# vlaxose/jstsp19

Hardware: AMD Instinct MI355X
Metric: channel-estimates/sec (batched MC) at Nt=Nr=64,K=64; NMSE vs ref (higher is better)
Workload: dtype c32 (storage and results fp32 complex; big contractions as split-f16 MFMA with fp32 accumulation, fp32-equivalent); 1 GPU; proposed_algorithm approximate Imax=100, Nt=Nr=64 Nrf=8 K=64 L=8 (N=64 M=4096 Gr=64 G2=512); Imax=100, outputs=S,Y,convergence_error, pilots=per-trial (B per trial), parallelism=trials sharded, dp1

## Files before the change

### jstsp19_amd/csrc/common.h

```cpp
#pragma once
#include <hip/hip_runtime.h>
#include <cstdint>
#include <cstdio>
#include <cstdarg>
#include <string>
#include <vector>
#include <map>
#include "../../include/jstsp.h"

namespace jstsp {

void set_error(const char *fmt, ...);

#define JSTSP_HIP(call)                                                                  \
    do {                                                                                 \
        hipError_t e_ = (call);                                                          \
        if (e_ != hipSuccess) {                                                          \
            jstsp::set_error("%s failed: %s (%s:%d)", #call, hipGetErrorString(e_),      \
                             __FILE__, __LINE__);                                        \
            return (int)e_;                                                              \
        }                                                                                \
    } while (0)

#define JSTSP_TRY(expr)                                                                  \
    do {                                                                                 \
        int rc_ = (expr);                                                                \
        if (rc_ != 0) return rc_;                                                        \
    } while (0)

#define JSTSP_REQUIRE(cond, code, ...)                                                   \
    do {                                                                                 \
        if (!(cond)) {                                                                   \
            jstsp::set_error(__VA_ARGS__);                                               \
            return (code);                                                               \
        }                                                                                \
    } while (0)

struct DeviceScope {
    int prev = -1;
    bool switched = false;
    hipError_t err = hipSuccess;
    explicit DeviceScope(int dev)
    {
        err = hipGetDevice(&prev);
        if (err == hipSuccess && prev != dev) {
            err = hipSetDevice(dev);
            switched = (err == hipSuccess);
        }
    }
    ~DeviceScope() { if (switched) (void)hipSetDevice(prev); }
    DeviceScope(const DeviceScope &) = delete;
    DeviceScope &operator=(const DeviceScope &) = delete;
};
struct Tuning {
    int h2 = 1;
    int fused = 1;
    int fused_parts = 0;
    int fused_kback = 4;
    int toeplitz = 2;
    int overlap = -1;
    int lanczos = 1;
    int lanczos_warm = 1;
    int lanczos_verify = 32;
    int eig128 = 1;
    int host_compact = 1;
    int host_pipeline = 1;
    int bj_mask = 1;
};
const Tuning &tune();
void load_tuning();

#define JSTSP_ENTER(ctx)                                                                 \
    jstsp::DeviceScope dev_scope_((ctx)->device);                                        \
    JSTSP_HIP(dev_scope_.err);                                                           \
    jstsp::load_tuning()

struct TrialParams {
    float rho, irho;
    float tauY_rho;
    float tauS_rho;
    float c_coef;
    float rho_lo, irho_lo, c_lo;
    float omc, omc_lo;
    float omr, omr_lo;
    float omir, omir_lo;
    float pad[2];
};
#if defined(__cplusplus)
inline TrialParams make_trial_params(double rho, double tau_Y, double tau_S)
{
    TrialParams p;
    auto split = [](double v, float &h, float &l) { h = (float)v; l = (float)(v - (double)h); };
    split(rho, p.rho, p.rho_lo);
    split(1.0 / rho, p.irho, p.irho_lo);
    split(rho / (rho + 1.0), p.c_coef, p.c_lo);
    split(1.0 / (rho + 1.0), p.omc, p.omc_lo);
    split(1.0 - rho, p.omr, p.omr_lo);
    split(1.0 - 1.0 / rho, p.omir, p.omir_lo);
    p.tauY_rho = (float)(tau_Y / rho);
    p.tauS_rho = (float)(tau_S / rho);
    p.pad[0] = p.pad[1] = 0.f;
    return p;
}
#if defined(__HIPCC__)
__device__ __forceinline__ float mul2(float ch, float cl, float x) { return fmaf(ch, x, cl * x); }
__device__ __forceinline__ float admm_v2(const TrialParams &p, float v2, float x, float xs)
{
    const float dx = x - xs;
    const float t = fmaf(-p.rho, dx, v2) - p.rho_lo * dx;
    return mul2(p.omc, p.omc_lo, t);
}
__device__ __forceinline__ float admm_x(const TrialParams &p, float v1, float y, float sy, float v2, float xs, float invd)
{
    const float ys = y + xs;
    return ((v1 + sy) + mul2(p.rho, p.rho_lo, ys) + mul2(p.omr, p.omr_lo, v2)) * invd;
}
__device__ __forceinline__ float admm_x2(const TrialParams &p, float v1, float y, float sy, float v2, float xs, float rh, float rl)
{
    const float ys = y + xs;
    const float s = (v1 + sy) + mul2(p.rho, p.rho_lo, ys) + mul2(p.omr, p.omr_lo, v2);
    return fmaf(s, rh, s * rl);
}
__device__ __forceinline__ void admm_invd(const TrialParams &p, float om, float &rh, float &rl)
{
    const float a = 2.f * p.rho, al = 2.f * p.rho_lo;
    const float dh = om + a;
    const float bb = dh - om;
    const float dl = ((om - (dh - bb)) + (a - bb)) + al;
    rh = __builtin_amdgcn_rcpf(dh);
    rl = rh * (fmaf(-dh, rh, 1.f) - dl * rh);
}
__device__ __forceinline__ float admm_k(const TrialParams &p, float x, float v2) { return fmaf(p.omir, v2, x) + p.omir_lo * v2; }
__device__ __forceinline__ float admm_v1(const TrialParams &p, float v1, float y, float x)
{
    const float d = y - x;
    return fmaf(p.rho, d, v1) + p.rho_lo * d;
}
__device__ __forceinline__ float admm_z(const TrialParams &p, float x, float v1) { return fmaf(-p.irho, v1, x) - p.irho_lo * v1; }
#endif
#endif

struct Arena {
    char *base = nullptr;
    size_t cap = 0, off = 0;
    int reserve(size_t bytes);
    void reset() { off = 0; }
    template <class T> T *get(size_t n) {
        size_t bytes = (n * sizeof(T) + 255) & ~size_t(255);
        if (off + bytes > cap) return nullptr;
        T *p = reinterpret_cast<T *>(base + off);
        off += bytes;
        return p;
    }
    void release();
};

struct ProfileSlot {
    int launches = 0;
    std::vector<std::pair<hipEvent_t, hipEvent_t>> pending;
    double total_ms = 0;
};

}

struct jstsp_ctx {
    int device = 0;
    hipStream_t stream = nullptr;
    bool own_stream = false;
    jstsp::Arena arena;
    bool profiling = false;
    std::map<std::string, jstsp::ProfileSlot> prof;
    std::vector<hipEvent_t> event_pool;
    int num_cus = 256;
    void *pinned = nullptr;
    size_t pinned_cap = 0, pinned_off = 0;
    hipEvent_t pinned_done = nullptr;
    bool pinned_pending = false;
    uint32_t *diag = nullptr;
    unsigned *lz_mismatch = nullptr;
    void *hpin = nullptr;
    size_t hpin_cap = 0;
    hipEvent_t hpin_done = nullptr;
    bool hpin_pending = false;
    int dict_block_hint = 0;
    int last_dict_block = 0;
    int fused_fallbacks = 0;
    float2 *unit = nullptr;
    double2 *unit64 = nullptr;
    jstsp_ctx *helper = nullptr;
    hipStream_t side[2] = {nullptr, nullptr};
    hipStream_t cu_stream[4] = {nullptr, nullptr, nullptr, nullptr};
    int cu_state = 0;
    hipStream_t bj_stream[3] = {nullptr, nullptr, nullptr};
    hipEvent_t bj_ev[6] = {nullptr, nullptr, nullptr, nullptr, nullptr, nullptr};
    hipEvent_t ev[10] = {nullptr, nullptr, nullptr, nullptr, nullptr, nullptr, nullptr, nullptr, nullptr, nullptr};
};

namespace jstsp {

struct GemmDesc {
    const float2 *A; long long sAt, sAi, sAk; int conjA;
    const float2 *B; long long sBt, sBk, sBj; int conjB;
    const float2 *B2;
    float2 *C; long long sCt; int ldc;
    const float2 *D; long long sDt; int ldd;
    float alpha, beta;
    int m, n, k, batch;
    int splitk; long long sCsplit;
    int epi;
    const TrialParams *prm;
    float2 *e_rw0, *e_w1, *e_w2, *e_w3;
// ... 115 lines not shown
```

### jstsp19_amd/csrc/proposed.hip

```cpp
#include "solver_common.h"
#include <cstdio>
#include <cmath>
#include <cstdlib>
#include <algorithm>

namespace jstsp {

struct ProposedWS {
    float2 *X, *V1, *V2, *C, *Xs, *Y, *ZK, *Zb, *Zb2;
    float *invD;
    float2 *V, *RV, *Res, *RRes, *S, *P1;
    float2 *Tc, *W;
    float2 *GA, *GB;
    TrialParams *prm;
    int32_t *rank;
    double *ce;
    float *lam;
    GramWS gz, gn;
    bool h2 = false;
    HPack Bc, Bs;
    uint32_t *kmax = nullptr, *wmax = nullptr;
    uint32_t *nmax = nullptr, *zmax = nullptr;
    bool h2g = false;
    HPack GBp;
// ... 274 lines not shown
        JSTSP_REQUIRE((PA || GAi) && (PB || GBi), JSTSP_E_NOMEM, "proposed_algorithm 'std': workspace exhausted");
        const size_t mark = ctx->arena.off;
        if (!PA) {
            JSTSP_TRY(hermitian_inverse(ctx, Gr, nA, w.GA, GAi));
            ctx->arena.off = mark;
            JSTSP_HIP(hipMemcpyAsync(w.GA, GAi, (size_t)nA * Gr * Gr * sizeof(float2), hipMemcpyDeviceToDevice, st));
        }
        if (!PB) {
            JSTSP_TRY(hermitian_inverse(ctx, G2, nB, w.GB, GBi));
            ctx->arena.off = mark;
            JSTSP_HIP(hipMemcpyAsync(w.GB, GBi, (size_t)nB * G2 * G2 * sizeof(float2), hipMemcpyDeviceToDevice, st));
        }
    }
    const long long snm = (long long)nm, sg = (long long)g, sng = (long long)ng;
    constexpr int rv_refresh = 4;
    auto refresh_at = [](int it) -> bool { return it % rv_refresh == 0; };
    const bool overlap = tn.overlap >= 0 ? tn.overlap != 0 : want_fused;
    uint32_t *const kmax0 = w.kmax;
    JSTSP_TRY(ensure_side_streams(ctx));
    hipStream_t sm = ctx->stream, s1 = overlap ? ctx->side[0] : sm, s2 = overlap ? ctx->side[1] : sm;
    hipEvent_t ev_x = ctx->ev[0], ev_svt = ctx->ev[1], ev_gxv = ctx->ev[2], ev_c = ctx->ev[3], ev_gv2 = ctx->ev[4],
               ev_ce = ctx->ev[5], ev_lxv = ctx->ev[6];
    if (Imax > 0) {
        JSTSP_TRY(launch_form_z(ctx, snm, batch, w.X, w.V1, w.prm, w.Zb));
        JSTSP_TRY(svt_prepare(ctx, w.gz, w.Zb, w.prm, nullptr, true));
    }
    const bool fz = w.gz.left;
    const bool hmax = w.h2 && fz && N <= 64;
    const bool zfly = hmax && want_ce && gram3_nsplit(N, M, G2, want_ce) > 0 && w.gz.nsplit == w.gn.nsplit;
    float2 *Zbuf[2] = {w.Zb, w.Zb2};
    const bool fusedp = want_fused && hmax && (want_ce ? zfly : true);
    const bool fusedy = fusedp;
    FusedWS fw;
    if (fusedp) {
        if (toep_env != 0 && !toep_probed) JSTSP_TRY(fused_probe_toeplitz(ctx, ctx->arena, B, strideB, G2, M, nB, &toep_gt));
        ctx->last_dict_block = toep_gt;
        JSTSP_TRY(fused_alloc(ctx->arena, fw, M, G2, nB, batch, fparts, toep_gt, toep_env >= 2 && fusedy));
        JSTSP_TRY(fused_pack_b(ctx, fw, B, strideB, G2, M, nB, w.Bc.bmax));
        JSTSP_HIP(hipMemsetAsync(fw.ovf, 0, (size_t)batch * sizeof(uint32_t), sm));
    }
    const int fused_kback = tn.fused_kback;
    bool passed = false;
    hipEvent_t ev_q1 = ctx->ev[7];
    if (want_ce) JSTSP_TRY(lanczos_warm_reset(ctx, w.gn));
    for (int it = 0; it < Imax; ++it) {
        if (want_ce) w.gn.lz.call = it;
        float2 *Zc = fz ? Zbuf[it & 1] : w.Zb, *Zn = fz ? Zbuf[(it + 1) & 1] : w.Zb;
        if (w.h2) {
            const size_t boff = (size_t)(it & 1) * 8 * (size_t)batch;
            w.kmax = kmax0 + boff; w.nmax = w.kmax + batch; w.zmax = w.kmax + 4 * (size_t)batch;
            w.wmax = w.kmax + 5 * (size_t)batch; w.pmax = w.kmax + 6 * (size_t)batch;
            if (!passed) JSTSP_HIP(hipMemsetAsync(w.kmax, 0, 8 * (size_t)batch * sizeof(uint32_t), sm));
        } else if (w.h2g) JSTSP_HIP(hipMemsetAsync(w.pmax, 0, 2 * (size_t)batch * sizeof(uint32_t), sm));
        int apply_no = 0;
        if (it > 0) JSTSP_HIP(hipStreamWaitEvent(sm, ev_svt, 0));
        if (it > 0 && want_ce) JSTSP_HIP(hipStreamWaitEvent(sm, ev_gxv, 0));
        if (passed) {
        } else if (fz) {
            JSTSP_TRY(launch_eye_minus(ctx, N, batch, w.gz.Q, w.gz.Q));
            GemmDesc dq = make_gemm('N', 'N', N, M, N, batch, Mat{w.gz.Q, (long long)N * N, N}, Mat{Zc, snm, N}, w.Y, snm, N);
            dq.epi = EPI_UPDATE_X; dq.prm = w.prm;
            dq.e_rw0 = w.V1; dq.e_w1 = w.X; dq.e_w2 = w.ZK;
            dq.e_r0 = w.V2; dq.e_r2 = w.Xs; dq.e_r3 = subY; dq.e_f0 = w.invD;
            dq.e_w3 = (it + 1 < Imax && (!zfly || fusedy)) ? Zn : nullptr;
            if (zfly && it > 0) { dq.B = w.X; dq.B2 = w.V1; }
            dq.epi_store_c = (it + 1 == Imax);
            if (w.h2) {
                dq.amax_out = w.kmax;
                if (N <= 64) { dq.amax_x = w.nmax; dq.amax_v1 = w.nmax + batch; dq.amax_z = w.zmax; }
            }
            JSTSP_TRY(launch_cgemm(ctx, dq, GEMM_MISC));
        } else {
            JSTSP_TRY(svt_apply(ctx, w.gz, Zc, w.Y));
            JSTSP_TRY(launch_update_x(ctx, snm, batch, w.X, w.V1, w.V2, w.C, w.Xs, w.Y, subY, w.invD, w.prm, w.ZK));
        }
        JSTSP_HIP(hipEventRecord(ev_x, sm));
        auto issue_s1 = [&](int stage) -> int {
            if (stage != 2) JSTSP_HIP(hipStreamWaitEvent(s1, ev_x, 0));
            StreamScope sc(ctx, s1);
            if (stage != 2 && !fz) JSTSP_TRY(launch_form_z(ctx, snm, batch, w.X, w.V1, w.prm, Zn));
            if (zfly) {
              if (stage != 2) {
                if (fusedp && it > 0) JSTSP_HIP(hipStreamWaitEvent(s1, ev_lxv, 0));
                JSTSP_TRY(launch_hgram3(ctx, w.X, w.V1, snm, N, M, batch, w.gz.nsplit, w.nmax, w.nmax + batch, w.zmax,
                                        w.prm, w.gz.Gpart, w.gn.Gpart, w.gn.Gpart + (size_t)batch * N * N * w.gn.nsplit));
                JSTSP_HIP(hipEventRecord(ev_gxv, s1));
                if (fusedp) {
                    JSTSP_HIP(hipStreamWaitEvent(s2, ev_gxv, 0));
                    StreamScope sc2(ctx, s2);
                    JSTSP_TRY(lmax_from_partials_range(ctx, w.gn, 0, 2 * batch, w.lam, true));
                    JSTSP_HIP(hipEventRecord(ev_lxv, s2));
                }
              }
              if (stage == 1) return 0;
                JSTSP_TRY(svt_prepare(ctx, w.gz, w.X, w.prm, nullptr, true, w.zmax, nullptr, true));
                if (fusedy) JSTSP_TRY(fused_pack_wq(ctx, fw, w.gz.Q, batch));
            } else {
                JSTSP_TRY(svt_prepare(ctx, w.gz, Zn, w.prm, nullptr, true, hmax ? w.zmax : nullptr));
                if (fusedy) JSTSP_TRY(fused_pack_wq(ctx, fw, w.gz.Q, batch));
            }
            JSTSP_HIP(hipEventRecord(ev_svt, s1));
            return 0;
        };
        const bool svt_split = passed && fusedp && zfly && it + 1 < Imax;
        if (it + 1 < Imax) JSTSP_TRY(issue_s1(svt_split ? 1 : 0));
        if (want_ce && !(zfly && it + 1 < Imax)) {
            JSTSP_HIP(hipStreamWaitEvent(s2, ev_x, 0));
            StreamScope sc(ctx, s2);
            JSTSP_TRY(gram_partials_range(ctx, w.gn, w.X, snm, 0, 2 * batch, hmax ? w.nmax : nullptr, nullptr, nullptr, true));
            JSTSP_HIP(hipEventRecord(ev_gxv, s2));
        }
        if (passed) {
            JSTSP_TRY(fused_reduce(ctx, fw, G2, M, batch, w.Tc));
        } else if (PB) {
            JSTSP_TRY(gemm(ctx, 'N', 'N', N, G2, M, batch, Mat{w.ZK, snm, N}, Mat{PB, strideB ? (long long)M * G2 : 0, M},
                           w.Tc, sng, N, 1.f, nullptr, 0, 0, 0.f, GEMM_CORRELATE));
        } else if (w.h2) {
            if (!fz) JSTSP_TRY(hgemm_absmax(ctx, w.ZK, snm, snm, batch, w.kmax));
            HGemmDesc hc{w.ZK, snm, N, w.kmax, w.Bc.data, strideB ? w.Bc.st : 0, w.Bc.bmax, strideB ? 1 : 0, w.Bc.KS,
                         w.Bc.JT, w.Tc, sng, N, N, G2, M, batch, EPI_NONE, nullptr, nullptr, nullptr};
            if (w.Kp.data && !strideB && w.Kp.KS == w.Bc.KS) {
                w.Kp.bmax = w.kmax;
                JSTSP_TRY(hgemm_repack(ctx, w.Kp, w.ZK, snm, N, 1, 0, M, N, w.kmax));
                hc.Ap = w.Kp.data; hc.sApt = w.Kp.st; hc.aKS = w.Kp.KS;
            }
            JSTSP_TRY(launch_hgemm(ctx, hc, "correlate"));
        } else
        JSTSP_TRY(gemm(ctx, 'N', 'C', N, G2, M, batch, Mat{w.ZK, snm, N}, Bm, w.Tc, sng, N, 1.f, nullptr, 0, 0,
                       0.f, GEMM_CORRELATE));
        const long long cnt_ll = std::min<long long>(10 + 5ll * (it + 1), (long long)g);
        const Mat GAl{GAlo, strideA ? (long long)Gr * Gr : 0, Gr};
        auto second_factor = [&](float2 *out, uint32_t *pm, bool exact) -> int {
            if (exact || !w.h2g) {
                GemmDesc dr = make_gemm('N', 'N', Gr, G2, G2, batch, Mat{w.P1, sg, Gr}, GBm, out, sg, Gr);
                dr.force_m64 = exact ? 1 : 0;
                return launch_cgemm(ctx, dr, GEMM_MISC);
            }
            HGemmDesc hg{w.P1, sg, Gr, pm, w.GBp.data, strideB ? w.GBp.st : 0, w.GBp.bmax, strideB ? 1 : 0,
                         w.GBp.KS, w.GBp.JT, out, sg, Gr, Gr, G2, G2, batch, EPI_NONE, nullptr, nullptr, nullptr};
            return launch_hgemm(ctx, hg, nullptr);
        };
        auto apply_R = [&](const float2 *Xin, float2 *out, bool exact) -> int {
            uint32_t *pm = w.pmax ? w.pmax + (size_t)(apply_no++ & 1) * batch : nullptr;
            if (exact) JSTSP_TRY(gemm(ctx, 'N', 'N', Gr, G2, Gr, batch, GAl, Mat{Xin, sg, Gr}, w.P1, sg, Gr));
            GemmDesc dp = make_gemm('N', 'N', Gr, G2, Gr, batch, GAm, Mat{Xin, sg, Gr}, w.P1, sg, Gr, 1.f, exact ? w.P1 : nullptr, sg,
                                    Gr, exact ? 1.f : 0.f);
            dp.amax_out = w.h2g ? pm : nullptr;
            JSTSP_TRY(launch_cgemm(ctx, dp, GEMM_MISC));
            return second_factor(out, pm, exact);
        };
        if (approx) {
            const bool refreshed = refresh_at(it);
            if (refreshed) JSTSP_TRY(apply_R(w.V, w.RV, true));
            GemmDesc dres = make_gemm('C', 'N', Gr, G2, N, batch, Am, Mat{w.Tc, sng, N}, w.Res, sg, Gr, 1.f, w.RV, sg, Gr, -1.f);
            JSTSP_TRY(launch_cgemm(ctx, dres, GEMM_MISC));
            JSTSP_TRY(apply_R(w.Res, w.RRes, false));
            if (svt_split) {
                JSTSP_HIP(hipEventRecord(ev_q1, sm));
                JSTSP_HIP(hipStreamWaitEvent(s1, ev_q1, 0));
                JSTSP_TRY(issue_s1(2));
            }
            JSTSP_TRY(launch_step_v(ctx, (int)g, batch, w.Res, w.RRes, w.V, w.S, w.rank, (int)cnt_ll, w.prm, w.ce,
                                    Imax, it, w.RV, svt_split));
        } else {
            float2 *left = PB ? w.V : w.P1;
            if (PA)
                JSTSP_TRY(gemm(ctx, 'N', 'N', Gr, G2, N, batch, Mat{PA, strideA ? (long long)Gr * N : 0, Gr},
                               Mat{w.Tc, sng, N}, left, sg, Gr));
            else {
                JSTSP_TRY(gemm(ctx, 'C', 'N', Gr, G2, N, batch, Am, Mat{w.Tc, sng, N}, w.Res, sg, Gr));
                JSTSP_TRY(gemm(ctx, 'N', 'N', Gr, G2, Gr, batch, GAm, Mat{w.Res, sg, Gr}, left, sg, Gr));
            }
            if (!PB) JSTSP_TRY(gemm(ctx, 'N', 'N', Gr, G2, G2, batch, Mat{w.P1, sg, Gr}, GBm, w.V, sg, Gr));
            JSTSP_TRY(launch_soft(ctx, (int)g, batch, w.V, w.S, w.rank, (int)cnt_ll, w.prm));
        }
        if (fusedp && !want_ce && it + 1 == Imax) break;
        if (w.h2) {
            GemmDesc dw = make_gemm('N', 'N', N, G2, Gr, batch, Am, Mat{w.S, sg, Gr}, w.W, sng, N);
            dw.amax_out = w.wmax;
            JSTSP_TRY(launch_cgemm(ctx, dw, GEMM_MISC));
        } else
        JSTSP_TRY(gemm(ctx, 'N', 'N', N, G2, Gr, batch, Am, Mat{w.S, sg, Gr}, w.W, sng, N));
        if (it > 0 && want_ce) JSTSP_HIP(hipStreamWaitEvent(sm, ev_gv2, 0));
        passed = false;
        if (fusedp && it + 1 < Imax) {
            uint32_t *nx = kmax0 + (size_t)((it + 1) & 1) * 8 * (size_t)batch;
            JSTSP_HIP(hipMemsetAsync(nx, 0, 8 * (size_t)batch * sizeof(uint32_t), sm));
            JSTSP_TRY(fused_pack_as(ctx, fw, w.W, sng, G2, M, batch, w.wmax));
            JSTSP_HIP(hipStreamWaitEvent(sm, ev_svt, 0));
            FusedDesc fd{fw.Bf, strideB ? fw.sBf : 0, w.Bc.bmax, strideB ? 1 : 0, fw.ASp, fw.sAS, w.wmax, w.kmax,
                         w.X, w.V1, w.V2, subY, w.Y, omega_direct ? Omega : w.invD, snm, w.prm, fw.Ppart,
                         nx, nx + batch, nx + 2 * (size_t)batch, nx + 4 * (size_t)batch, w.nmax + 2 * (size_t)batch, fw.ovf,
                         M, G2, batch, fparts,
                         fusedy ? fw.Wqp : nullptr, Zbuf[(it + 1) & 1], w.zmax,
                         (fw.v2 && zfly) ? nullptr : Zbuf[it & 1],
                         (fusedy && it + 2 == Imax) ? w.Y : nullptr, fused_kback,
                         fw.Ec, strideB ? fw.sEc : 0, fw.gt ? 31 - __builtin_clz((unsigned)fw.gt) : 0, fw.ecols, fw.ehalo,
                         fw.v2, fw.XsD, fw.Kf, omega_direct ? 1 : 0};
            JSTSP_TRY(launch_fused_pass(ctx, fd));
            passed = true;
        } else
        if (w.h2) {
            JSTSP_TRY(hgemm_repack(ctx, w.Wp, w.W, sng, N, 1, 0, G2, N, w.wmax));
            if (!w.Bs.data)
                JSTSP_TRY(hgemm_pack(ctx, w.Bs, ctx->arena, B, strideB, 1, G2, 0, G2, M, nB, (long long)G2 * M, w.Bc.bmax));
            HGemmDesc hs{w.W, sng, N, w.wmax, w.Bs.data, strideB ? w.Bs.st : 0, w.Bs.bmax, strideB ? 1 : 0, w.Bs.KS,
                         w.Bs.JT, w.Xs, snm, N, N, M, G2, batch, fz ? EPI_UPDATE_C : EPI_NONE, w.prm, w.X, w.V2,
                         hmax ? w.nmax + 2 * (size_t)batch : nullptr, w.Wp.data, w.Wp.st, w.Wp.KS};
            JSTSP_TRY(launch_hgemm(ctx, hs, "synthesize"));
            if (!fz) JSTSP_TRY(launch_update_c(ctx, snm, batch, w.X, w.Xs, w.V2, w.C, w.prm));
        } else if (fz) {
            GemmDesc ds = make_gemm('N', 'N', N, M, G2, batch, Mat{w.W, sng, N}, Bm, w.Xs, snm, N);
            ds.epi = EPI_UPDATE_C; ds.prm = w.prm;
            ds.e_r0 = w.X; ds.e_rw0 = w.V2;
            JSTSP_TRY(launch_cgemm(ctx, ds, GEMM_SYNTH));
        } else {
            JSTSP_TRY(gemm(ctx, 'N', 'N', N, M, G2, batch, Mat{w.W, sng, N}, Bm, w.Xs, snm, N, 1.f, nullptr, 0, 0,
                           0.f, GEMM_SYNTH));
            JSTSP_TRY(launch_update_c(ctx, snm, batch, w.X, w.Xs, w.V2, w.C, w.prm));
        }
        if (want_ce) {
            JSTSP_HIP(hipEventRecord(ev_c, sm));
            JSTSP_HIP(hipStreamWaitEvent(s2, ev_c, 0));
            if (zfly) JSTSP_HIP(hipStreamWaitEvent(s2, ev_gxv, 0));
            StreamScope sc(ctx, s2);
            JSTSP_TRY(gram_partials_range(ctx, w.gn, w.X, snm, 2 * batch, batch, hmax ? w.nmax : nullptr, nullptr, nullptr, true));
            JSTSP_HIP(hipEventRecord(ev_gv2, s2));
            if (fusedp && zfly && it + 1 < Imax) JSTSP_TRY(lmax_from_partials_range(ctx, w.gn, 2 * batch, batch, w.lam, true));
            else JSTSP_TRY(lmax_from_partials(ctx, w.gn, w.lam, true));
            JSTSP_TRY(launch_ce_ratio(ctx, batch, w.lam + batch, w.lam + 2 * batch, w.lam, w.ce, Imax, it));
            JSTSP_HIP(hipEventRecord(ev_ce, s2));
        }
    }
    if (want_ce && Imax > 0) JSTSP_HIP(hipStreamWaitEvent(sm, ev_ce, 0));
    if (defer) {
        defer->active = true; defer->fused = fusedp; defer->want_ce = want_ce && Imax > 0; defer->batch = batch; defer->g = g; defer->nm = nm;
        defer->Imax = Imax; defer->dS = w.S; defer->dY = w.Y; defer->dce = w.ce; defer->ovf = fusedp ? fw.ovf : nullptr;
        return 0;
    }

    JSTSP_TRY(stage_out(ctx, reinterpret_cast<float2 *>(S_out), w.S, batch * g, memspace));
    JSTSP_TRY(stage_out(ctx, reinterpret_cast<float2 *>(Y_out), w.Y, batch * nm, memspace));
    if (want_ce && Imax > 0) JSTSP_TRY(stage_out(ctx, ce_out, w.ce, (size_t)batch * 3 * Imax, memspace));
    if (fusedp && overflowed) {
        std::vector<uint32_t> flags(batch);
        JSTSP_HIP(hipMemcpyAsync(flags.data(), fw.ovf, (size_t)batch * sizeof(uint32_t), hipMemcpyDeviceToHost, st));
        JSTSP_HIP(hipStreamSynchronize(st));
        for (int t = 0; t < batch; ++t)
            if (flags[t]) overflowed->push_back(t);
    }
    if (memspace == JSTSP_HOST) {
        JSTSP_HIP(hipStreamSynchronize(st));
        if (!approx) JSTSP_TRY(diag_check_host(ctx, "proposed_algorithm 'std'"));
    }
    return 0;
}

static int resolve_overflowed(jstsp_ctx *ctx, const std::vector<int> &ovf, int N, int M, int Gr, int G2, const jstsp_c32 *subY,
                              const float *Omega, const jstsp_c32 *A, long long strideA, const jstsp_c32 *B, long long strideB,
                              int Imax, const double *tau_Y, const double *tau_S, const double *rho, int type,
                              const int32_t *indx_S, jstsp_c32 *S_out, jstsp_c32 *Y_out, double *ce_out, int memspace, int *count)
{
    const size_t nm = (size_t)N * M, g = (size_t)Gr * G2;
    for (size_t i = 0; i < ovf.size();) {
        size_t j = i + 1;
        while (j < ovf.size() && ovf[j] == ovf[j - 1] + 1) ++j;
        const int t0 = ovf[i], cnt = (int)(j - i);
        JSTSP_TRY(proposed_impl(ctx, N, M, Gr, G2, cnt, subY + t0 * nm, Omega + t0 * nm, A + (size_t)t0 * strideA, strideA,
                                B + (size_t)t0 * strideB, strideB, Imax, tau_Y + t0, tau_S + t0, rho + t0, type,
                                indx_S ? indx_S + t0 * g : nullptr, S_out + t0 * g, Y_out ? Y_out + t0 * nm : nullptr,
                                ce_out ? ce_out + (size_t)t0 * 3 * Imax : nullptr, memspace, false, nullptr));
        *count += cnt;
        i = j;
    }
    return 0;
}

static int proposed_finish(jstsp_ctx *ctx, const PendingSolve &p, jstsp_c32 *S_out, jstsp_c32 *Y_out, double *ce_out, std::vector<int> *ovf)
{
    JSTSP_ENTER(ctx);
    JSTSP_TRY(stage_out(ctx, reinterpret_cast<float2 *>(S_out), p.dS, p.batch * p.g, JSTSP_HOST));
    JSTSP_TRY(stage_out(ctx, reinterpret_cast<float2 *>(Y_out), p.dY, p.batch * p.nm, JSTSP_HOST));
    if (p.want_ce) JSTSP_TRY(stage_out(ctx, ce_out, p.dce, (size_t)p.batch * 3 * p.Imax, JSTSP_HOST));
    std::vector<uint32_t> flags(p.ovf ? p.batch : 0);
    if (p.ovf) JSTSP_HIP(hipMemcpyAsync(flags.data(), p.ovf, (size_t)p.batch * sizeof(uint32_t), hipMemcpyDeviceToHost, ctx->stream));
    JSTSP_HIP(hipStreamSynchronize(ctx->stream));
    for (int t = 0; t < (int)flags.size(); ++t)
        if (flags[t]) ovf->push_back(t);
    return 0;
}

extern "C" int jstsp_proposed_algorithm_c32(jstsp_ctx *ctx, int N, int M, int Gr, int G2, int batch,
                                            const jstsp_c32 *subY, const float *Omega,
                                            const jstsp_c32 *A, long long strideA, const jstsp_c32 *B,
                                            long long strideB, int Imax, const double *tau_Y,
                                            const double *tau_S, const double *rho, int type,
                                            const int32_t *indx_S, jstsp_c32 *S_out, jstsp_c32 *Y_out,
                                            double *ce_out, int memspace)
{
    std::vector<int> ovf;
    if (ctx) { ctx->fused_fallbacks = 0; ctx->last_dict_block = 0; }
    const size_t nm = (size_t)N * M, g = (size_t)Gr * G2;
    const size_t in_bytes = (size_t)batch * (nm * 12 + (strideB ? (size_t)G2 * M * 8 : 0));
    const bool pipeline = ctx && memspace == JSTSP_HOST && type == JSTSP_TYPE_APPROXIMATE && batch >= 128 && Imax > 1 && Y_out &&
                          in_bytes >= ((size_t)256 << 20) && subY && Omega && A && B && tau_Y && tau_S && rho && S_out &&
                          tune_host_pipeline();
    if (pipeline) {
        if (!ctx->helper) JSTSP_TRY(jstsp_create(ctx->device, &ctx->helper));
        jstsp_ctx *cx[2] = {ctx, ctx->helper};
// ... 160 lines not shown
```

### jstsp19_amd/csrc/runtime.hip

```cpp
#include "solver_common.h"
#include <cstring>
#include <cmath>
#include <cstdlib>
#include <algorithm>

namespace jstsp {

static thread_local char g_err[512] = "";

static thread_local Tuning g_tune;
const Tuning &tune() { return g_tune; }

static int env_int(const char *name, int dflt)
{
    const char *e = getenv(name);
    return (e && *e) ? atoi(e) : dflt;
}

void load_tuning()
{
    Tuning t;
    t.h2 = env_int("JSTSP_H2", t.h2);
    t.fused = env_int("JSTSP_FUSED", t.fused);
    t.fused_parts = env_int("JSTSP_FUSED_PARTS", t.fused_parts);
    t.fused_kback = env_int("JSTSP_FUSED_KBACK", t.fused_kback);
    t.toeplitz = env_int("JSTSP_TOEPLITZ", t.toeplitz);
    t.overlap = env_int("JSTSP_OVERLAP", t.overlap);
    t.lanczos = env_int("JSTSP_LANCZOS", t.lanczos);
    t.lanczos_warm = env_int("JSTSP_LANCZOS_WARM", t.lanczos_warm);
    t.lanczos_verify = env_int("JSTSP_LANCZOS_VERIFY", t.lanczos_verify);
    t.eig128 = env_int("JSTSP_EIG128", t.eig128);
    t.bj_mask = env_int("JSTSP_BJ_MASK", t.bj_mask);
    t.host_pipeline = env_int("JSTSP_HOST_PIPELINE", t.host_pipeline);
    t.host_compact = env_int("JSTSP_HOST_COMPACT", t.host_compact);
    g_tune = t;
}

void set_error(const char *fmt, ...)
{
    va_list ap;
    va_start(ap, fmt);
    vsnprintf(g_err, sizeof(g_err), fmt, ap);
    va_end(ap);
}

int Arena::reserve(size_t bytes)
{
    if (bytes <= cap) return 0;
    if (base) {
        JSTSP_HIP(hipDeviceSynchronize());
        JSTSP_HIP(hipFree(base));
        base = nullptr;
        cap = 0;
    }
    size_t want = bytes + (bytes >> 4) + (1u << 20);
    hipError_t e = hipMalloc((void **)&base, want);
    if (e != hipSuccess) {
        (void)hipGetLastError();
        want = bytes;
        e = hipMalloc((void **)&base, want);
    }
    if (e != hipSuccess) {
        (void)hipGetLastError();
        base = nullptr;
        set_error("workspace allocation of %zu bytes failed: %s", bytes, hipGetErrorString(e));
        return JSTSP_E_NOMEM;
    }
    cap = want;
    return 0;
}

void Arena::release()
{
    if (base) (void)hipFree(base);
    base = nullptr;
    cap = off = 0;
}

static hipEvent_t take_event(jstsp_ctx *ctx)
{
    if (!ctx->event_pool.empty()) {
        hipEvent_t e = ctx->event_pool.back();
        ctx->event_pool.pop_back();
        return e;
    }
    hipEvent_t e = nullptr;
    (void)hipEventCreate(&e);
    return e;
}

void prof_begin(jstsp_ctx *ctx, const char *name)
{
    if (!ctx->profiling) return;
    ProfileSlot &s = ctx->prof[name];
    hipEvent_t a = take_event(ctx), b = take_event(ctx);
    (void)hipEventRecord(a, ctx->stream);
    s.pending.emplace_back(a, b);
}

void prof_end(jstsp_ctx *ctx, const char *name)
{
    if (!ctx->profiling) return;
    ProfileSlot &s = ctx->prof[name];
    (void)hipEventRecord(s.pending.back().second, ctx->stream);
    s.launches++;
}

static void prof_collect(jstsp_ctx *ctx)
{
    for (auto &kv : ctx->prof) {
        for (auto &pr : kv.second.pending) {
            float ms = 0.f;
            (void)hipEventSynchronize(pr.second);
            if (hipEventElapsedTime(&ms, pr.first, pr.second) == hipSuccess) kv.second.total_ms += ms;
            ctx->event_pool.push_back(pr.first);
            ctx->event_pool.push_back(pr.second);
        }
        kv.second.pending.clear();
    }
}

GemmDesc make_gemm(char opA, char opB, int m, int n, int k, int batch, Mat A, Mat B, float2 *C, long long sCt,
                   int ldc, float alpha, const float2 *D, long long sDt, int ldd, float beta, int splitk,
                   long long sCsplit)
{
    GemmDesc d;
    d.A = A.p; d.sAt = A.st;
    const bool tA = (opA == 'T' || opA == 'C'), tB = (opB == 'T' || opB == 'C');
    d.conjA = (opA == 'C' || opA == 'J');
    d.conjB = (opB == 'C' || opB == 'J');
    if (!tA) { d.sAi = 1; d.sAk = A.ld; } else { d.sAi = A.ld; d.sAk = 1; }
    d.B = B.p; d.sBt = B.st; d.B2 = nullptr;
    if (!tB) { d.sBk = 1; d.sBj = B.ld; } else { d.sBk = B.ld; d.sBj = 1; }
    d.C = C; d.sCt = sCt; d.ldc = ldc;
    d.D = D; d.sDt = sDt; d.ldd = ldd;
    d.alpha = alpha; d.beta = beta;
    d.m = m; d.n = n; d.k = k; d.batch = batch;
    d.splitk = splitk < 1 ? 1 : splitk; d.sCsplit = sCsplit;
    d.epi = EPI_NONE; d.prm = nullptr; d.e_rw0 = d.e_w1 = d.e_w2 = d.e_w3 = nullptr;
    d.e_r0 = d.e_r1 = d.e_r2 = d.e_r3 = nullptr; d.e_f0 = nullptr; d.epi_store_c = 1; d.amax_out = nullptr; d.amax_x = d.amax_v1 = d.amax_z = nullptr;
    d.force_m64 = 0; d.C_lo = nullptr; d.herm_upper = 0;
    d.sa_mode = 0; d.sa_lr = d.sa_lt = nullptr; d.sa_rho = d.sa_thr = 0.f;
    return d;
}

int gemm(jstsp_ctx *ctx, char opA, char opB, int m, int n, int k, int batch, Mat A, Mat B, float2 *C,
         long long sCt, int ldc, float alpha, const float2 *D, long long sDt, int ldd, float beta, int tag,
         int splitk, long long sCsplit)
{
    return launch_cgemm(ctx, make_gemm(opA, opB, m, n, k, batch, A, B, C, sCt, ldc, alpha, D, sDt, ldd, beta, splitk,
                                       sCsplit), tag);
}

static int pick_nsplit(int n, int kc, int batch)
{
    const int tiles = ((n + 63) / 64) * ((n + 63) / 64);
    long long want = (1024 + (long long)batch * tiles - 1) / ((long long)batch * tiles);
    const int kmax = std::max(1, kc / 256);
    want = std::max<long long>(1, std::min<long long>(want, kmax));
    return (int)std::min<long long>(want, 32);
}

size_t GramWS::bytes(int rows, int cols, int batch, bool need_q, int force_nsplit)
{
    const int n = std::min(rows, cols), kc = std::max(rows, cols);
    const int ns = force_nsplit > 0 ? force_nsplit : pick_nsplit(n, kc, batch);
    size_t b = rnd256((size_t)batch * ns * n * n * sizeof(float2));
    if (!need_q && n <= 128) b += rnd256((size_t)batch * lanczos_ne(n) * sizeof(float2)) + rnd256((size_t)batch * sizeof(int));
    if (need_q) {
        b += rnd256((size_t)batch * n * n * sizeof(float2));
        if (n <= 64) b += rnd256((size_t)batch * eig_fast_ne(n) * eig_fast_ne(n) * sizeof(float2));
        else b += 2 * rnd256((size_t)batch * n * n * sizeof(float2));
        if (n > 64 && eig_needs_global_v(n)) {
            const int ne = (n + 1) & ~1;
            b += rnd256((size_t)batch * ne * ne * sizeof(float2));
        }
    }
    return b;
// ... 432 lines not shown
```

### jstsp19_amd/csrc/solver_common.h

```cpp
#pragma once
#include "common.h"
#include <vector>

namespace jstsp {

struct Mat {
    const float2 *p; long long st; int ld;
};

int gemm(jstsp_ctx *ctx, char opA, char opB, int m, int n, int k, int batch, Mat A, Mat B, float2 *C,
         long long sCt, int ldc, float alpha = 1.f, const float2 *D = nullptr, long long sDt = 0,
         int ldd = 0, float beta = 0.f, int tag = GEMM_MISC, int splitk = 1, long long sCsplit = 0);

int gram_f64(jstsp_ctx *ctx, char side, const float2 *X, long long sXt, int rows, int cols, int count, float2 *G, long long sGt,
             float2 *Glo = nullptr);

bool grad_head_shape_ok(int N, int Gr, int G2);
int launch_grad_head(jstsp_ctx *ctx, int G2, int batch, const float2 *P, long long sPt, long long sPp, int parts, const float2 *Kf,
                     const float2 *Bdl, long long sBdl, const float2 *A, long long sA, const float2 *GA, long long sGA,
                     const float2 *RV, float2 *Tc, float2 *Res, float2 *P1, uint32_t *pmax);

GemmDesc make_gemm(char opA, char opB, int m, int n, int k, int batch, Mat A, Mat B, float2 *C, long long sCt,
                   int ldc, float alpha = 1.f, const float2 *D = nullptr, long long sDt = 0, int ldd = 0,
                   float beta = 0.f, int splitk = 1, long long sCsplit = 0);

struct GramWS {
    int rows = 0, cols = 0, n = 0, nsplit = 1, batch = 0;
    bool left = true;
    float2 *Gpart = nullptr;
    float2 *Q = nullptr;
    float2 *Vg = nullptr;
    float2 *Uwarm = nullptr;
    float2 *Twarm = nullptr;
    mutable int warm = 0;
    float eig_stop = 0.f;
    mutable LanczosWarm lz;
    static size_t bytes(int rows, int cols, int batch, bool need_q, int force_nsplit = 0);
    int alloc(Arena &a, int rows, int cols, int batch, bool need_q, int force_nsplit = 0);
};

int gram_partials(jstsp_ctx *ctx, const GramWS &w, const float2 *Z, long long sZt);
int svt_batched(jstsp_ctx *ctx, const GramWS &w, const float2 *Z, const TrialParams *prm,
                const float *tau, float2 *Y, bool sequence = false);
int svt_prepare(jstsp_ctx *ctx, const GramWS &w, const float2 *Z, const TrialParams *prm, const float *tau,
                bool sequence, const uint32_t *amax = nullptr, const float2 *Z2 = nullptr,
                bool gram_done = false);
int svt_apply(jstsp_ctx *ctx, const GramWS &w, const float2 *Z, float2 *Y);
int gram_partials_range(jstsp_ctx *ctx, const GramWS &w, const float2 *Z, long long sZt, int t0, int count,
                        const uint32_t *amax = nullptr, const float2 *Z2 = nullptr,
                        const TrialParams *zprm = nullptr, bool norm_only = false);
int lanczos_warm_reset(jstsp_ctx *ctx, const GramWS &w);
int lmax_from_partials(jstsp_ctx *ctx, const GramWS &w, float *lam, bool lanczos = false);
int lmax_from_partials_range(jstsp_ctx *ctx, const GramWS &w, int first, int count, float *lam, bool lanczos);
int ensure_side_streams(jstsp_ctx *ctx);
int ensure_bj_resources(jstsp_ctx *ctx);
bool ensure_cu_streams(jstsp_ctx *ctx);
struct StreamScope {
    jstsp_ctx *c; hipStream_t saved;
    StreamScope(jstsp_ctx *ctx, hipStream_t s) : c(ctx), saved(ctx->stream) { c->stream = s; }
    ~StreamScope() { c->stream = saved; }
};
int sigma_max_sq(jstsp_ctx *ctx, const GramWS &w, const float2 *Z, float *lam, bool lanczos = false);

size_t hinv_bytes(int n, int count);
int hermitian_inverse(jstsp_ctx *ctx, int n, int count, const float2 *G, float2 *Ginv);

bool pinv_fits(int rows, int cols);
int launch_pinv(jstsp_ctx *ctx, int rows, int cols, int count, const float2 *A, long long sAt, int lda, float2 *P,
                long long sPt, int ldp, float *rcond_out = nullptr);
int ensure_diag(jstsp_ctx *ctx);
int diag_reset(jstsp_ctx *ctx);
int diag_check_host(jstsp_ctx *ctx, const char *what);

struct PendingSolve {
    bool active = false, fused = false, want_ce = false;
    int batch = 0;
    size_t g = 0, nm = 0;
    int Imax = 0;
    const float2 *dS = nullptr, *dY = nullptr;
    const double *dce = nullptr;
    const uint32_t *ovf = nullptr;
};
int proposed_enqueue_device(jstsp_ctx *ctx, int N, int M, int Gr, int G2, int batch, const jstsp_c32 *subY, const float *Omega,
                            const jstsp_c32 *A, long long strideA, const jstsp_c32 *B, long long strideB, int Imax,
                            const double *tau_Y, const double *tau_S, const double *rho, int type, const int32_t *indx_S,
                            bool want_ce, PendingSolve *out);
int proposed_pending_flags(jstsp_ctx *ctx, const PendingSolve &p, std::vector<int> *ovf);
int proposed_resolve_device(jstsp_ctx *ctx, int N, int M, int Gr, int G2, int batch, const jstsp_c32 *subY, const float *Omega,
                            const jstsp_c32 *A, long long strideA, const jstsp_c32 *B, long long strideB, int Imax,
                            const double *tau_Y, const double *tau_S, const double *rho, int type, const int32_t *indx_S,
                            jstsp_c32 *S_dev, jstsp_c32 *Y_dev, double *ce_dev);

int upload(jstsp_ctx *ctx, void *dst, const void *src, size_t bytes);

template <class T> int stage_in(jstsp_ctx *ctx, const T *src, size_t n, int memspace, const T **out)
{
    if (memspace == JSTSP_DEVICE) { *out = src; return 0; }
    T *d = ctx->arena.get<T>(n);
    JSTSP_REQUIRE(d, JSTSP_E_NOMEM, "workspace exhausted while staging an input");
    JSTSP_HIP(hipMemcpyAsync(d, src, n * sizeof(T), hipMemcpyHostToDevice, ctx->stream));
    *out = d;
    return 0;
}
template <class T> int stage_out(jstsp_ctx *ctx, T *dst, const T *dev, size_t n, int memspace)
{
    if (!dst) return 0;
    JSTSP_HIP(hipMemcpyAsync(dst, dev, n * sizeof(T),
                             memspace == JSTSP_DEVICE ? hipMemcpyDeviceToDevice : hipMemcpyDeviceToHost,
                             ctx->stream));
    return 0;
}
inline size_t rnd256(size_t b) { return (b + 255) & ~size_t(255); }

template <class T>
int host_toeplitz_stage(jstsp_ctx *ctx, const T *Bh, int G2, int M, int nB, float2 *Bdev, float2 *Cdev, size_t cdev_elems, int *gt_out);
size_t host_toeplitz_compact_elems(int G2, int M, int nB);

struct FusedWS {
    uint4 *Bf = nullptr; long long sBf = 0;
    uint4 *ASp = nullptr; long long sAS = 0;
    float2 *Ppart = nullptr;
    uint32_t *ovf = nullptr;
    uint4 *Wqp = nullptr;
    int parts = 0;
    uint4 *Ec = nullptr; long long sEc = 0;
    int gt = 0, ecols = 0, ehalo = 0;
    int v2 = 0;
    const float2 *Bsrc = nullptr; long long sBsrc = 0;
    float2 *Bdl = nullptr; long long sBdl = 0;
    float2 *XsD = nullptr, *Kf = nullptr;
};
struct FusedDesc {
    const uint4 *Bf; long long sBf;
    const uint32_t *bmax; int sbmax;
    const uint4 *ASp; long long sAS;
    const uint32_t *wmax;
    const uint32_t *kmax_prev;
    float2 *X, *V1, *V2;
    const float2 *subY, *Y; const float *invD;
    long long snm;
    const TrialParams *prm;
    float2 *Ppart;
    uint32_t *kmax_out, *xmax, *v1max, *zmax, *v2max, *ovf;
    int M, G2, batch, parts;
    const uint4 *Wqp; const float2 *Zin; const uint32_t *zmax_in; float2 *Zout, *Yout;
    int kback;
    const uint4 *Ec; long long sEc; int gsh, ecols, ehalo;
    int v2; const float2 *XsD; float2 *Kf;
    int inv_is_omega;
};
bool fused_shape_ok(int N, int M, int G2, int parts);
size_t fused_bytes(int M, int G2, int nB, int batch, int parts);
int fused_probe_toeplitz(jstsp_ctx *ctx, Arena &ar, const float2 *B, long long sBt, int G2, int M, int nB, int *gt);
int toeplitz_gram_assemble(jstsp_ctx *ctx, const float2 *B, long long sBt, int G2, int M, int gt, int nB, const float2 *G0,
                           const float2 *G0lo, float2 *G, float2 *Glo);
int fused_alloc(Arena &ar, FusedWS &f, int M, int G2, int nB, int batch, int parts, int gt, int v2);
int fused_pack_b(jstsp_ctx *ctx, FusedWS &f, const float2 *B, long long sBt, int G2, int M, int nB, const uint32_t *bmax);
int fused_pack_as(jstsp_ctx *ctx, const FusedWS &f, const float2 *W, long long sWt, int G2, int M, int batch, const uint32_t *wmax);
int launch_fused_pass(jstsp_ctx *ctx, const FusedDesc &d);
int fused_reduce(jstsp_ctx *ctx, const FusedWS &f, int G2, int M, int batch, float2 *Tc);
int fused_pack_wq(jstsp_ctx *ctx, const FusedWS &f, const float2 *Q, int batch);

}
```

Baseline: 827.1 channel-estimates/s.

## Fuse residual GEMM and first R-factor GEMM into one MFMA kernel

Adds a kernel that computes Res = A^H*Tc - RV for a 64-column tile, keeps the result in shared memory, multiplies it by GA to produce P1 and its per-trial amax, then hands off to the existing second factor. This replaces two separate complex GEMM launches and removes the global round trip of Res before the P1 product. The kernel uses fp32 MFMA with an XCD-aware trial mapping and applies only for N=Gr=64 when the split SVT path and h2g are active. It is gated by a tuning flag, which can be turned off with JSTSP_FUSED=2.

```diff
diff --git a/jstsp19_amd/csrc/common.h b/jstsp19_amd/csrc/common.h
--- a/jstsp19_amd/csrc/common.h
+++ b/jstsp19_amd/csrc/common.h
@@ -57,6 +57,7 @@
     int fused = 1;
     int fused_parts = 0;
     int fused_kback = 4;
+    int grad_fused = 1;
     int toeplitz = 2;
     int overlap = -1;
     int lanczos = 1;
diff --git a/jstsp19_amd/csrc/gradstep.hip b/jstsp19_amd/csrc/gradstep.hip
--- /dev/null
+++ b/jstsp19_amd/csrc/gradstep.hip
@@ -0,0 +1,142 @@
+#include "solver_common.h"
+
+namespace jstsp {
+
+namespace {
+
+typedef float f32x16 __attribute__((ext_vector_type(16)));
+
+constexpr int GK = 16;
+constexpr int GLD = 65;
+
+__global__ __launch_bounds__(256) void grad_res_p1_kernel(const float2 *A, long long sAt, const float2 *Tc, const float2 *RV,
+                                                          float2 *Res, const float2 *GA, long long sGAt, float2 *P1,
+                                                          uint32_t *pmax, int G2, int batch)
+{
+    __shared__ float2 smem[4 * GK * GLD];
+    const int tiles = G2 / 64;
+    const int xcd = blockIdx.x & 7, slot = blockIdx.x >> 3;
+    const int t = (slot / tiles) * 8 + xcd;
+    if (t >= batch) return;
+    const int n0 = (slot % tiles) * 64;
+
+    const int tid = threadIdx.x, lane = tid & 63, wave = tid >> 6;
+    const int wi = wave & 1, wj = wave >> 1, l31 = lane & 31, lhi = lane >> 5;
+    const float2 *Ap = A + (long long)t * sAt;
+    const long long cbase = (long long)t * 64 * G2 + 64ll * n0;
+    const float2 *Tp = Tc + cbase;
+    float2 *sA = smem, *sB = smem + 2 * GK * GLD;
+
+    const int pk = tid & 15, pr = tid >> 4;
+    float2 ra[4], rb[4];
+    auto gload = [&](int k0) {
+#pragma unroll
+        for (int p = 0; p < 4; ++p) {
+            ra[p] = Ap[k0 + pk + 64 * (pr + 16 * p)];
+            rb[p] = Tp[k0 + pk + 64 * (pr + 16 * p)];
+        }
+    };
+    auto sstore = [&](int buf) {
+#pragma unroll
+        for (int p = 0; p < 4; ++p) {
+            sA[buf * GK * GLD + pk * GLD + pr + 16 * p] = make_float2(ra[p].x, -ra[p].y);
+            sB[buf * GK * GLD + pk * GLD + pr + 16 * p] = rb[p];
+        }
+    };
+
+    f32x16 are, aim;
+#pragma unroll
+    for (int r = 0; r < 16; ++r) { are[r] = 0.f; aim[r] = 0.f; }
+
+    gload(0);
+    sstore(0);
+    __syncthreads();
+    for (int kt = 0; kt < 64 / GK; ++kt) {
+        const int buf = kt & 1;
+        const bool refresh = kt + 1 < 64 / GK;
+        if (refresh) gload((kt + 1) * GK);
+        const float2 *a = sA + buf * GK * GLD + wi * 32 + l31;
+        const float2 *bb = sB + buf * GK * GLD + wj * 32 + l31;
+        float2 av = a[lhi * GLD], bv = bb[lhi * GLD];
+#pragma unroll
+        for (int kp = 0; kp < GK / 2; ++kp) {
+            float2 an = av, bn = bv;
+            if (kp + 1 < GK / 2) {
+                const int kr = 2 * (kp + 1) + lhi;
+                an = a[kr * GLD];
+                bn = bb[kr * GLD];
+            }
+            are = __builtin_amdgcn_mfma_f32_32x32x2f32(bv.x, av.x, are, 0, 0, 0);
+            aim = __builtin_amdgcn_mfma_f32_32x32x2f32(bv.x, av.y, aim, 0, 0, 0);
+            are = __builtin_amdgcn_mfma_f32_32x32x2f32(-bv.y, av.y, are, 0, 0, 0);
+            aim = __builtin_amdgcn_mfma_f32_32x32x2f32(bv.y, av.x, aim, 0, 0, 0);
+            av = an; bv = bn;
+        }
+        if (refresh) sstore(buf ^ 1);
+        __syncthreads();
+    }
+
+    const int gi = wi * 32 + l31;
+    const float2 *Gp = GA + (long long)t * sGAt + gi + 64 * lhi;
+    float2 ga[8];
+#pragma unroll
+    for (int q = 0; q < 8; ++q) ga[q] = Gp[128 * q];
+#pragma unroll
+    for (int r = 0; r < 16; ++r) {
+        const int j = wj * 32 + (r & 3) + 8 * (r >> 2) + 4 * lhi;
+        const long long ix = cbase + gi + 64ll * j;
+        const float2 dv = RV[ix];
+        const float2 o = make_float2(are[r] - dv.x, aim[r] - dv.y);
+        Res[ix] = o;
+        smem[gi * GLD + j] = o;
+        are[r] = 0.f; aim[r] = 0.f;
+    }
+    __syncthreads();
+
+    const float2 *rs = smem + wj * 32 + l31;
+#pragma unroll
+    for (int c = 0; c < 4; ++c) {
+        float2 gn[8];
+#pragma unroll
+        for (int q = 0; q < 8; ++q) gn[q] = (c < 3) ? Gp[128 * (8 * (c + 1) + q)] : ga[q];
+#pragma unroll
+        for (int q = 0; q < 8; ++q) {
+            const int kp = 8 * c + q;
+            const float2 av = ga[q], bv = rs[(2 * kp + lhi) * GLD];
+            are = __builtin_amdgcn_mfma_f32_32x32x2f32(bv.x, av.x, are, 0, 0, 0);
+            aim = __builtin_amdgcn_mfma_f32_32x32x2f32(bv.x, av.y, aim, 0, 0, 0);
+            are = __builtin_amdgcn_mfma_f32_32x32x2f32(-bv.y, av.y, are, 0, 0, 0);
+            aim = __builtin_amdgcn_mfma_f32_32x32x2f32(bv.y, av.x, aim, 0, 0, 0);
+        }
+#pragma unroll
+        for (int q = 0; q < 8; ++q) ga[q] = gn[q];
+    }
+    float tmax = 0.f;
+#pragma unroll
+    for (int r = 0; r < 16; ++r) {
+        const int j = wj * 32 + (r & 3) + 8 * (r >> 2) + 4 * lhi;
+        P1[cbase + gi + 64ll * j] = make_float2(are[r], aim[r]);
+        tmax = fmaxf(tmax, fmaxf(fabsf(are[r]), fabsf(aim[r])));
+    }
+#pragma unroll
+    for (int o = 32; o > 0; o >>= 1) tmax = fmaxf(tmax, __shfl_xor(tmax, o));
+    if (lane == 0) atomicMax(&pmax[t], __float_as_uint(tmax));
+}
+
+}
+
+bool grad_fused_shape(int N, int Gr, int G2) { return N == 64 && Gr == 64 && G2 >= 64 && G2 % 64 == 0; }
+
+int launch_grad_res_p1(jstsp_ctx *ctx, const float2 *A, long long sAt, const float2 *Tc, const float2 *RV, float2 *Res,
+                       const float2 *GA, long long sGAt, float2 *P1, uint32_t *pmax, int G2, int batch)
+{
+    JSTSP_REQUIRE(G2 >= 64 && G2 % 64 == 0 && batch > 0 && pmax, JSTSP_E_ARG, "gradient step: fused Res / P1 launch at G2 = %d", G2);
+    const long long grid = (long long)((batch + 7) / 8) * 8 * (G2 / 64);
+    JSTSP_REQUIRE(grid < (1ll << 31), JSTSP_E_UNSUPPORTED, "gradient step: grid too large");
+    hipLaunchKernelGGL(grad_res_p1_kernel, dim3((unsigned)grid), dim3(256), 0, ctx->stream, A, sAt, Tc, RV, Res, GA, sGAt, P1,
+                       pmax, G2, batch);
+    JSTSP_HIP(hipGetLastError());
+    return 0;
+}
+
+}
diff --git a/jstsp19_amd/csrc/proposed.hip b/jstsp19_amd/csrc/proposed.hip
--- a/jstsp19_amd/csrc/proposed.hip
+++ b/jstsp19_amd/csrc/proposed.hip
@@ -450,9 +450,16 @@
         if (approx) {
             const bool refreshed = refresh_at(it);
             if (refreshed) JSTSP_TRY(apply_R(w.V, w.RV, true));
+            if (svt_split && tn.grad_fused != 0 && w.h2g && grad_fused_shape(N, Gr, G2)) {
+                uint32_t *pm = w.pmax + (size_t)(apply_no++ & 1) * batch;
+                JSTSP_TRY(launch_grad_res_p1(ctx, A, strideA, w.Tc, w.RV, w.Res, w.GA, strideA ? (long long)Gr * Gr : 0, w.P1, pm,
+                                             G2, batch));
+                JSTSP_TRY(second_factor(w.RRes, pm, false));
+            } else {
             GemmDesc dres = make_gemm('C', 'N', Gr, G2, N, batch, Am, Mat{w.Tc, sng, N}, w.Res, sg, Gr, 1.f, w.RV, sg, Gr, -1.f);
             JSTSP_TRY(launch_cgemm(ctx, dres, GEMM_MISC));
             JSTSP_TRY(apply_R(w.Res, w.RRes, false));
+            }
             if (svt_split) {
                 JSTSP_HIP(hipEventRecord(ev_q1, sm));
                 JSTSP_HIP(hipStreamWaitEvent(s1, ev_q1, 0));
diff --git a/jstsp19_amd/csrc/runtime.hip b/jstsp19_amd/csrc/runtime.hip
--- a/jstsp19_amd/csrc/runtime.hip
+++ b/jstsp19_amd/csrc/runtime.hip
@@ -24,6 +24,7 @@
     t.fused = env_int("JSTSP_FUSED", t.fused);
     t.fused_parts = env_int("JSTSP_FUSED_PARTS", t.fused_parts);
     t.fused_kback = env_int("JSTSP_FUSED_KBACK", t.fused_kback);
+    t.grad_fused = t.fused == 2 ? 0 : 1;
     t.toeplitz = env_int("JSTSP_TOEPLITZ", t.toeplitz);
     t.overlap = env_int("JSTSP_OVERLAP", t.overlap);
     t.lanczos = env_int("JSTSP_LANCZOS", t.lanczos);
diff --git a/jstsp19_amd/csrc/solver_common.h b/jstsp19_amd/csrc/solver_common.h
--- a/jstsp19_amd/csrc/solver_common.h
+++ b/jstsp19_amd/csrc/solver_common.h
@@ -161,4 +161,8 @@
 int fused_reduce(jstsp_ctx *ctx, const FusedWS &f, int G2, int M, int batch, float2 *Tc);
 int fused_pack_wq(jstsp_ctx *ctx, const FusedWS &f, const float2 *Q, int batch);
 
+bool grad_fused_shape(int N, int Gr, int G2);
+int launch_grad_res_p1(jstsp_ctx *ctx, const float2 *A, long long sAt, const float2 *Tc, const float2 *RV, float2 *Res,
+                       const float2 *GA, long long sGAt, float2 *P1, uint32_t *pmax, int G2, int batch);
+
 }
```

Result: faster. 835.6 channel-estimates/s, median of 6 (+1.0%).
